# google/lasr

Hardware: AMD Instinct MI355X
Metric: rasterizer fwd+bwd frames/sec at 256x256, 2.3k faces (higher is better)
Workload: dtype f32

## Files before the change

### lasr_amd/csrc/sr_backward.h

```cpp
#pragma once
#include "sr_common.h"

namespace lasr {

constexpr bool BWD_FM = true;
constexpr int QCAP = 128;
constexpr int BWD_THREADS = 64;

template <bool LASR_FAST, int NCH, bool WIDE = false>
__global__ __launch_bounds__(BWD_THREADS)
__attribute__((amdgpu_waves_per_eu(LASR_FAST && NCH == 3 && !WIDE ? 6 : 1, LASR_FAST && NCH == 3 && !WIDE ? 7 : 8)))
void sr_backward_kernel(RasterArgs A, const float* __restrict__ colors,
                                                          const float* __restrict__ aggrs,
                                                          const float* __restrict__ gcolors,
                                                          float* __restrict__ gfaces, float* __restrict__ gtex)
{
    __shared__ unsigned int s_ring[BWD_THREADS / 64][QCAP];
    __shared__ __attribute__((aligned(16))) float s_rec[BWD_THREADS / 64][REC + (LASR_FAST ? BX : 0)];
    constexpr bool FM = BWD_FM;
    const Modes m = LASR_FAST ? Modes{2, 1, 2, 1, 1} : A.m;
    if (A.near_far_dev) { A.near = A.near_far_dev[0]; A.far = A.near_far_dev[1]; }
    const int lane = threadIdx.x & 63;
    unsigned int* ring = s_ring[threadIdx.x >> 6];
    int blk;
    {
        const int total = gridDim.x, per = total >> 3;
        blk = (total & 7) == 0 ? (blockIdx.x & 7) * per + (per - 1 - (blockIdx.x >> 3)) : total - 1 - blockIdx.x;
    }
    const int ext_src = LASR_FAST ? (int)k_bwd_ext_tbl[lane] : 0;
    const int gw = __builtin_amdgcn_readfirstlane((int)((blk * blockDim.x + threadIdx.x) >> 6));
    if (gw >= A.N * A.F) return;
    const int bn = face_div(gw, A.fdiv_m, A.fdiv_s), fn = gw - bn * A.F;
    const int IS = A.IS, P = IS * IS;
    const cptr_t rec = as_const(A.recs + (size_t)gw * REC);
    const cptr_t tex = as_const(A.textures + (size_t)gw * A.T * NCH);
    const int flags = __float_as_int(rec[R_FLAGS]);
    typedef const float __attribute__((address_space(3)))* lptr_t;
    if (LASR_FAST && (flags & 16)) {
        float* dst = s_rec[threadIdx.x >> 6];
        if (lane < REC) dst[lane] = A.recs[(size_t)gw * REC + lane];
        dst[REC + lane] = bwd_ext_word_tbl(A.recs + (size_t)gw * REC, flags, lane, ext_src);
        __builtin_amdgcn_wave_barrier();
    }
    const lptr_t lrec = (lptr_t)s_rec[threadIdx.x >> 6];

    const unsigned rlo = (unsigned)__float_as_int(rec[R_BB + 0]), rext = (unsigned)__float_as_int(rec[R_BB + 1]);
    const int x0 = (int)(rlo & 0xffff), r0 = (int)(rlo >> 16);
    const int bw = (int)(rext & 0xffff) + 1, bh = (int)(rext >> 16) + 1;
    const bool empty = rlo == 0xffffffffu;
    const int npx = empty ? 0 : bw * bh;

    float gv[9] = {0, 0, 0, 0, 0, 0, 0, 0, 0};
    constexpr int NGT = 3 * NCH < 18 ? 18 : 3 * NCH;
    constexpr int THIRD = NCH == 9 ? 18 : 0;
    float gt[NGT];
#pragma unroll
    for (int k = 0; k < NGT; k++) gt[k] = 0.f;
    const bool front = (flags & 8) != 0;
    const bool vertex_tex = (m.tex == 1);
    const int lim = (A.N * A.F - gw) * A.T;
    const bool use_far = (m.dist == 2) && (flags & 16);
    const float inv_is = A.inv_is;
    const bool pow2 = (IS & (IS - 1)) == 0;
    const float cx_a = A.cx_a, cx_b = A.cx_b, cy_b = A.cy_b;
    auto centre_x = [&](int xi) { return pow2 ? __builtin_fmaf((float)xi, cx_a, cx_b) : pix_center_p2(xi, IS, inv_is, pow2); };
    auto centre_y = [&](int row) { return pow2 ? __builtin_fmaf((float)row, -cx_a, cy_b) : pix_center_p2(IS - 1 - row, IS, inv_is, pow2); };
    float ld[9];
    const float far_t = A.far_t;
    if (use_far) {
#pragma unroll
        for (int k = 0; k < 3; k++) {
            const float h = __builtin_amdgcn_sqrtf(rec[R_HK2 + k]);
            ld[3 * k] = rec[R_INV + 3 * k] * h; ld[3 * k + 1] = rec[R_INV + 3 * k + 1] * h; ld[3 * k + 2] = rec[R_INV + 3 * k + 2] * h;
        }
    }
    const float tie_scale = rec[R_TIE];
    bool depth_safe = false;
    if (flags & 16) {
        const float z0 = rec[R_FACE + 2], z1 = rec[R_FACE + 5], z2 = rec[R_FACE + 8];
        const float zlo = fminf(fminf(z0, z1), z2), zhi = fmaxf(fmaxf(z0, z1), z2);
        depth_safe = zlo > 0.f && zlo * (1.f - 1e-4f) > A.near && zhi * (1.f + 1e-4f) < A.far;
    }
    constexpr int GC = 0, CO = 1, AG = 2;
    const unsigned P4 = (unsigned)P * 4u;

    int r = 0, c = 0;
    const int walk = __float_as_int(rec[15]);
    const int dr = empty ? 0 : walk >> 17, dc = empty ? 0 : 64 - dr * bw;
    if (!empty) { r = (lane * (walk & 0x1ffff)) >> 16; c = lane - r * bw; }

    int head = 0, tail = 0, base = 0;
    gplane_t pb[3];
    if (!WIDE) {
        pb[GC] = plane_base(gcolors, (size_t)bn * (NCH + 1), P);
        pb[CO] = plane_base(colors, (size_t)bn * (NCH + 1), P);
        pb[AG] = plane_base(aggrs, (size_t)bn * 2, P);
    }
    auto ld_plane = [&](const float* tensor, int which, int nplanes, int plane, int pn_, unsigned off_) -> float {
#if defined(LASR_BWD_ABL) && LASR_BWD_ABL == 3
        return 0.25f + 1e-3f * (float)(pn_ & 255) + 0.01f * (float)plane;
#endif
        if (WIDE) return tensor[((size_t)bn * nplanes + plane) * P + pn_];
        return ld_plane_at(pb[which], off_ + (unsigned)plane * P4);
    };
    while (true) {
        if (base < npx) {
            const int xi = x0 + c, row = r0 + r;
            const bool in_range = base + lane < npx;
            c += dc; r += dr;
            if (c >= bw) { c -= bw; r += 1; }
            base += 64;
            bool keep = in_range;
            if (use_far) {
                const float xp = __builtin_fmaf((float)xi, cx_a, cx_b), yp = __builtin_fmaf((float)row, -cx_a, cy_b);
                const float d0 = __builtin_fmaf(ld[0], xp, __builtin_fmaf(ld[1], yp, ld[2]));
                const float d1 = __builtin_fmaf(ld[3], xp, __builtin_fmaf(ld[4], yp, ld[5]));
                const float d2 = __builtin_fmaf(ld[6], xp, __builtin_fmaf(ld[7], yp, ld[8]));
                keep = in_range && !(fminf(fminf(d0, d1), d2) < far_t);
            }
            const unsigned long long mask = wave_mask(keep);
            if (keep) ring[(tail + bits_below_lane(mask)) & (QCAP - 1)] = (unsigned)xi | ((unsigned)row << 16);
            tail += __popcll(mask);
        }
        const int avail = tail - head;
        if (!(avail >= 64 || (base >= npx && avail > 0))) {
            if (base >= npx) break;
            continue;
        }
        __builtin_amdgcn_wave_barrier();
        const bool active = lane < avail;
        const unsigned int packed = ring[(head + lane) & (QCAP - 1)];
        head += min(avail, 64);
#if defined(LASR_BWD_ABL) && LASR_BWD_ABL == 1
        gv[0] += (float)packed;
        continue;
#endif
        if (!active) continue;
        const int xi = packed & 0xffff, row = packed >> 16;
        const int pn = row * IS + xi;
        unsigned po = (unsigned)pn << 2;
        const float xp = centre_x(xi), yp = centre_y(row);

        float w0, w1, w2;
        Frag fr;
        if (LASR_FAST && (flags & 16)) {
            if (!fragment_one_ext(lrec, lrec + REC, flags, A.thr, A.sigma, xp, yp, w0, w1, w2, fr, tie_scale)) continue;
        } else
        if (!fragment<FM, cptr_t, LASR_FAST>(rec, m.dist, A.thr, A.sigma, xp, yp, w0, w1, w2, fr)) continue;
        const float D = fr.D;
#if defined(LASR_BWD_ABL) && LASR_BWD_ABL == 2
        gv[0] += D + fr.dx + fr.dy + fr.t0 + fr.t1 + fr.t2 + fr.sign;
        continue;
#endif

        float Ca = ld_plane(gcolors, GC, NCH + 1, NCH, pn, po);
        if (m.alpha == 1) Ca = div_<FM>(Ca, (float)A.F);
        else if (m.alpha == 2) {
            const float a_out = ld_plane(colors, CO, NCH + 1, NCH, pn, po);
            Ca *= div_<FM>(1 - a_out, fmaxf(1 - D, 1e-6f));
        }
        float C = Ca;

        const float u0 = w0, u1 = w1, u2 = w2;
        if (vertex_tex) clip_normalise<FM, LASR_FAST>(w0, w1, w2); else clip_normalise<false>(w0, w1, w2);
        const float iz0r = rec[R_IZ + 0], iz1r = rec[R_IZ + 1], iz2r = rec[R_IZ + 2];
        const float q0 = w0 * iz0r, q1 = w1 * iz1r, q2 = w2 * iz2r;
        const float zp = LASR_FAST ? __builtin_amdgcn_rcpf(q0 + q1 + q2) : depth_at<FM>(rec, w0, w1, w2);
        if (!depth_safe) {
            float zc = zp;
            const float tol = 1e-4f * fabsf(zp);
            if (fabsf(zp - A.near) <= tol || fabsf(zp - A.far) <= tol) zc = depth_forward_exact(rec, xp, yp);
            if (zc < A.near || zc > A.far) continue;
        }

        float gz0 = 0, gz1 = 0, gz2 = 0;
        auto reenter = [&]() { if (!WIDE) asm volatile("" : "+v"(po)); };
        if (m.rgb == 0) {
            reenter();
            if ((float)fn == ld_plane(aggrs, AG, 2, 1, pn, po)) {
                reenter();
                float g[NCH];
#pragma unroll
                for (int k = 0; k < NCH; k++) g[k] = ld_plane(gcolors, GC, NCH + 1, k, pn, po);
                if (vertex_tex) {
#pragma unroll
                    for (int k = 0; k < NCH; k++) {
                        gt[k] += w0 * g[k]; gt[NCH + k] += w1 * g[k]; gt[2 * NCH + k] += w2 * g[k];
                    }
                } else {
                    const int j = surface_texel(w0, w1, A.res);
                    if (j >= 0 && j < A.T) {
                        float* gtp = gtex + (size_t)gw * A.T * 3 + 3 * j;
                        atomicAdd(gtp + 0, g[0]); atomicAdd(gtp + 1, g[1]); atomicAdd(gtp + 2, g[2]);
                    }
                }
            }
        } else if (front || m.double_side) {
            reenter();
            const float ssum = ld_plane(aggrs, AG, 2, 0, pn, po);
            const float smax = ld_plane(aggrs, AG, 2, 1, pn, po);
            const float zn = div_<FM>(A.far - zp, A.far - A.near);
            const float sm = div_<FM>(D * exp_<FM>(div_<FM>(zn - smax, A.gamma)), ssum);
            float g[NCH];
#pragma unroll
            for (int k = 0; k < NCH; k++) g[k] = ld_plane(gcolors, GC, NCH + 1, k, pn, po);
            if (vertex_tex) {
#pragma unroll
                for (int k = 0; k < NCH; k++) {
                    gt[k] += sm * (w0 * g[k]); gt[NCH + k] += sm * (w1 * g[k]); gt[2 * NCH + k] += sm * (w2 * g[k]);
                }
            } else {
                const int j = surface_texel(w0, w1, A.res);
                if (j >= 0 && j < A.T) {
                    float* gtp = gtex + (size_t)gw * A.T * 3 + 3 * j;
                    atomicAdd(gtp + 0, sm * g[0]); atomicAdd(gtp + 1, sm * g[1]); atomicAdd(gtp + 2, sm * g[2]);
                }
            }
            float Crgb = 0.f;
#pragma unroll
            for (int k = 0; k < NCH; k++)
                Crgb += g[k] * (sample_colour(tex, w0, w1, w2, A.res, k, m.tex, lim, NCH) - ld_plane(colors, CO, NCH + 1, k, pn, po));
            Crgb *= sm;
            C += div_<FM>(Crgb, D);
            const float Cz = div_<FM>(div_<FM>(Crgb, A.gamma), A.near - A.far) * zp * zp;
            if (LASR_FAST) {
                gz0 = Cz * q0 * iz0r; gz1 = Cz * q1 * iz1r; gz2 = Cz * q2 * iz2r;
            } else {
                const float iz0 = __builtin_amdgcn_rcpf(rec[R_FACE + 2]), iz1 = __builtin_amdgcn_rcpf(rec[R_FACE + 5]), iz2 = __builtin_amdgcn_rcpf(rec[R_FACE + 8]);
                gz0 = Cz * w0 * iz0 * iz0;
                gz1 = Cz * w1 * iz1 * iz1;
                gz2 = Cz * w2 * iz2 * iz2;
            }
        }

        C *= div_<FM>(D * (1 - D), A.sigma);
        float gx0 = 0, gy0 = 0, gx1 = 0, gy1 = 0, gx2 = 0, gy2 = 0;
        if (m.dist == 1) {
            const float t0 = fr.t0, t1 = fr.t1, t2 = fr.t2;
            const int p = t0 > t1 ? (t1 > t2 ? 2 : 1) : (t0 > t2 ? 2 : 0);
            const float ipx = rec[R_INV + 3 * p + 0], ipy = rec[R_INV + 3 * p + 1];
            const float dis = fr.dis;
            const float sc = 2.f * sqrtf(fabsf(dis));
            float gxy[3][2];
#pragma unroll
            for (int l = 0; l < 2; l++) {
                const float ipl = l == 0 ? ipx : ipy;
#pragma unroll
                for (int k = 0; k < 3; k++) {
                    float acc = 0.f;
                    acc += -ipl * rec[R_INV + 3 * k + 0] * xp;
                    acc += -ipl * rec[R_INV + 3 * k + 1] * yp;
                    acc += -ipl * rec[R_INV + 3 * k + 2] * 1.f;
                    gxy[k][l] = acc * C * sc;
                }
            }
            gx0 = gxy[0][0]; gy0 = gxy[0][1]; gx1 = gxy[1][0]; gy1 = gxy[1][1]; gx2 = gxy[2][0]; gy2 = gxy[2][1];
        } else if (m.dist == 2) {
            const float k2 = 2 * fr.sign * C;
            gx0 = k2 * (fr.t0 + u0) * fr.dx; gy0 = k2 * (fr.t0 + u0) * fr.dy;
            gx1 = k2 * (fr.t1 + u1) * fr.dx; gy1 = k2 * (fr.t1 + u1) * fr.dy;
            gx2 = k2 * (fr.t2 + u2) * fr.dx; gy2 = k2 * (fr.t2 + u2) * fr.dy;
        }
        gv[0] += gx0; gv[1] += gy0; gv[2] += gz0;
        gv[3] += gx1; gv[4] += gy1; gv[5] += gz1;
        gv[6] += gx2; gv[7] += gy2; gv[8] += gz2;
    }

    float v18[18], red[5];
    const int lane_row = lane >> 4;
    const int sub = lane_row == 0 ? 0 : lane_row == 1 ? 2 : lane_row == 2 ? 1 : 3;
    float* gf = gfaces + (size_t)gw * 9;
    float* gtp = gtex + (size_t)gw * 3 * NCH;
#pragma unroll
    for (int pass = 0; pass < (NCH > 3 ? 2 : 1); pass++) {
#pragma unroll
        for (int k = 0; k < 9; k++) {
            v18[k] = pass == 0 ? gv[k] : (vertex_tex ? gt[9 + k] : 0.f);
            v18[9 + k] = pass == 0 ? (vertex_tex ? gt[k] : 0.f) : (NCH == 9 && vertex_tex ? gt[THIRD + k] : 0.f);
        }
        wave_reduce18(v18, red);
        if ((lane & 15) == 15) {
#pragma unroll
            for (int i = 0; i < 5; i++) {
                if (i == 4 && (lane_row & 1)) continue;
                const int comp = i == 4 ? 16 + (lane_row >> 1) : 4 * i + sub;
                const bool ow = A.overwrite_grads && vertex_tex;
                if (pass == 0) {
                    if (comp < 9) gf[comp] = ow ? red[i] : gf[comp] + red[i];
                    else if (vertex_tex) gtp[comp - 9] = ow ? red[i] : gtp[comp - 9] + red[i];
                } else if ((comp < 9 || NCH == 9) && vertex_tex) gtp[9 + comp] = ow ? red[i] : gtp[9 + comp] + red[i];
            }
        }
    }
}

}
```

### lasr_amd/csrc/sr_device.h

```cpp
#pragma once
#include <hip/hip_runtime.h>

namespace lasr {

constexpr int REC = 48;

constexpr int R_BB = 0, R_FLAGS = 2, R_INV = 3, R_HK2 = 12, R_FACE = 16, R_DEN = 25, R_IDEN = 28, R_TIE = 31, R_E = 32, R_IZ = 41;

typedef const float __attribute__((address_space(4)))* cptr_t;
__device__ __forceinline__ cptr_t as_const(const float* p) { return (cptr_t)(unsigned long long)p; }

typedef const char __attribute__((address_space(1)))* gplane_t;
__device__ __forceinline__ gplane_t plane_base(const float* tensor, size_t plane, int P)
{
    unsigned long long u = (unsigned long long)(tensor + plane * (size_t)P);
    asm volatile("" : "+s"(u));
    return (gplane_t)u;
}
__device__ __forceinline__ float ld_plane_at(gplane_t base, unsigned byte_offset)
{
    return *(const float __attribute__((address_space(1)))*)(base + byte_offset);
}

struct Modes {
    int dist, rgb, alpha, tex, double_side;
};

__device__ __forceinline__ float pix_center(int i, int is)
{
    return (float)(2 * i + 1 - is) / (float)is;
}

__device__ __forceinline__ bool recip_safe(float b)
{
    const float m = fabsf(b);
    return m > 1e-18f && m < 1e18f;
}
__device__ __forceinline__ float div_by_recip(float a, float b, float y)
{
    float q = a * y;
    float e = __builtin_fmaf(-b, q, a);
    q = __builtin_fmaf(e, y, q);
    e = __builtin_fmaf(-b, q, a);
    return __builtin_fmaf(e, y, q);
}

__device__ __forceinline__ float recip_noscale(float x)
{
    float y = __builtin_amdgcn_rcpf(x);
    y = __builtin_fmaf(__builtin_fmaf(-x, y, 1.f), y, y);
    float q = y;
    q = __builtin_fmaf(__builtin_fmaf(-x, q, 1.f), y, q);
    return __builtin_fmaf(__builtin_fmaf(-x, q, 1.f), y, q);
}
__device__ __forceinline__ double recip64_noscale(double x)
{
    double y = __builtin_amdgcn_rcp(x);
    y = __builtin_fma(__builtin_fma(-x, y, 1.), y, y);
    y = __builtin_fma(__builtin_fma(-x, y, 1.), y, y);
    const double q = y;
    return __builtin_fma(__builtin_fma(-x, q, 1.), y, q);
}

__device__ __forceinline__ float max_finite(float a, float b)
{
    float r;
    asm("v_max_f32 %0, %1, %2" : "=v"(r) : "v"(a), "v"(b));
    return r;
}

typedef unsigned short u16x2_t __attribute__((ext_vector_type(2)));
__device__ __forceinline__ bool rect_has(int lo, int ext, int pxy)
{
    const u16x2_t d = __builtin_bit_cast(u16x2_t, pxy) - __builtin_bit_cast(u16x2_t, lo);
    const u16x2_t m = __builtin_elementwise_min(d, __builtin_bit_cast(u16x2_t, ext));
    return __builtin_bit_cast(int, m) == __builtin_bit_cast(int, d);
}

__device__ __forceinline__ int first_pixel_ge(float lo, int IS)
{
    if (lo != lo) return 0;
    const float e = ceilf((lo * (float)IS + (float)IS - 1.f) * 0.5f);
    int i = e < 0.f ? 0 : (e > (float)IS ? IS : (int)e);
    for (int k = 0; k < 4 && i > 0 && pix_center(i - 1, IS) >= lo; k++) i--;
    for (int k = 0; k < 4 && i < IS && pix_center(i, IS) < lo; k++) i++;
    return i;
}
__device__ __forceinline__ int last_pixel_le(float hi, int IS)
{
    if (hi != hi) return IS - 1;
    const float e = floorf((hi * (float)IS + (float)IS - 1.f) * 0.5f);
    int i = e < -1.f ? -1 : (e > (float)(IS - 1) ? IS - 1 : (int)e);
    for (int k = 0; k < 4 && i < IS - 1 && pix_center(i + 1, IS) <= hi; k++) i++;
    for (int k = 0; k < 4 && i >= 0 && pix_center(i, IS) > hi; k++) i--;
    return i;
}

__device__ __forceinline__ float pix_center_p2(int i, int is, float inv_is, bool pow2)
{
    return pow2 ? (float)(2 * i + 1 - is) * inv_is : pix_center(i, is);
}

__host__ __device__ __forceinline__ float near_tie_scale(float h2a, float h2b, float h2c);

__device__ __forceinline__ void build_record(const float* __restrict__ f, float* __restrict__ rec,
                                             short4* __restrict__ rect, float margin, int IS,
                                             float* __restrict__ info27)
{
    const float x0 = f[0], y0 = f[1], x1 = f[3], y1 = f[4], x2 = f[6], y2 = f[7];
    float adj[9];
    adj[0] = y1 - y2; adj[1] = x2 - x1; adj[2] = x1 * y2 - x2 * y1;
    adj[3] = y2 - y0; adj[4] = x0 - x2; adj[5] = x2 * y0 - x0 * y2;
    adj[6] = y0 - y1; adj[7] = x1 - x0; adj[8] = x0 * y1 - x1 * y0;
    float det = x2 * (y0 - y1) + x0 * (y1 - y2) + x1 * (y2 - y0);
    if (det > 0) { double d = (double)det; det = (float)(d > 1e-10 ? d : 1e-10); }
    else         { double d = (double)det; det = (float)(d < -1e-10 ? d : -1e-10); }
    float inv[9], sym[9];
#pragma unroll
    for (int k = 0; k < 9; k++) inv[k] = adj[k] / det;
#pragma unroll
    for (int j = 0; j < 3; j++)
#pragma unroll
        for (int k = 0; k < 3; k++) sym[3 * j + k] = f[3 * j] * f[3 * k] + f[3 * j + 1] * f[3 * k + 1] + 1;
    int flags = 0;
    {
        const float px[3] = {x0, x1, x2}, py[3] = {y0, y1, y2};
#pragma unroll
        for (int k = 0; k < 3; k++) {
            const int b = (k + 1) % 3, c = (k + 2) % 3;
            const bool obt = (px[b] - px[k]) * (px[c] - px[k]) + (py[b] - py[k]) * (py[c] - py[k]) < 0;
            if (obt && (flags & 7) == 0) flags |= 1 << k;
        }
    }
    if ((y2 - y0) * (x1 - x0) < (y1 - y0) * (x2 - x0)) flags |= 8;
#pragma unroll
    for (int k = 0; k < 9; k++) rec[R_FACE + k] = f[k];
#pragma unroll
    for (int k = 0; k < 9; k++) rec[R_INV + k] = inv[k];
#pragma unroll
    for (int k = 0; k < 3; k++) {
        const int b = (k + 1) % 3;
        float e[3];
#pragma unroll
        for (int j = 0; j < 3; j++) { e[j] = sym[3 * k + j] - sym[3 * b + j]; rec[R_E + 3 * k + j] = e[j]; }
        rec[R_DEN + k] = e[k] - e[b];
    }
    {
        const float det0 = x2 * (y0 - y1) + x0 * (y1 - y2) + x1 * (y2 - y0);
        const float px[3] = {x0, x1, x2}, py[3] = {y0, y1, y2};
        bool ok = true;
#pragma unroll
        for (int k = 0; k < 3; k++) {
            const int b = (k + 1) % 3, c = (k + 2) % 3;
            const float ex = px[c] - px[b], ey = py[c] - py[b];
            const float l2 = ex * ex + ey * ey;
            const float h2 = l2 > 0.f ? det0 * det0 / l2 : 0.f;
            rec[R_HK2 + k] = h2;
            ok = ok && (h2 > 1e-4f) && (h2 < 1e4f) && (l2 < 16.f);
        }
        if (ok) flags |= 16;
    }
    rec[R_FLAGS] = __int_as_float(flags);
    const float xmax = fmaxf(fmaxf(x0, x1), x2) + margin, xmin = fminf(fminf(x0, x1), x2) - margin;
    const float ymax = fmaxf(fmaxf(y0, y1), y2) + margin, ymin = fminf(fminf(y0, y1), y2) - margin;
    int px0 = first_pixel_ge(xmin, IS), px1 = last_pixel_le(xmax, IS);
    const int yi0 = first_pixel_ge(ymin, IS), yi1 = last_pixel_le(ymax, IS);
    int r0 = IS - 1 - yi1, r1 = IS - 1 - yi0;
    if (px0 > px1 || r0 > r1) { px0 = 32767; px1 = -1; r0 = 32767; r1 = -1; }
    *rect = make_short4((short)px0, (short)px1, (short)r0, (short)r1);
    if (px0 > px1) { rec[R_BB + 0] = __int_as_float(-1); rec[R_BB + 1] = __int_as_float(0); }
    else {
        rec[R_BB + 0] = __int_as_float((px0 & 0xffff) | (r0 << 16));
        rec[R_BB + 1] = __int_as_float(((px1 - px0) & 0xffff) | ((r1 - r0) << 16));
    }
    {
        bool ok = true;
#pragma unroll
        for (int k = 0; k < 3; k++) {
            const float d = rec[R_DEN + k], z = f[3 * k + 2];
            rec[R_IDEN + k] = 1.f / d;
            rec[R_IZ + k] = 1.f / z;
            ok = ok && recip_safe(d) && z >= 1e-6f && z <= 1e6f;
        }
#pragma unroll
        for (int k = 0; k < 9; k++) ok = ok && fabsf(inv[k]) < 1e30f;
        if (ok) rec[R_FLAGS] = __int_as_float(__float_as_int(rec[R_FLAGS]) | 32);
        {
            const int bw = px0 > px1 ? 1 : px1 - px0 + 1;
            const int mdiv = bw < 64 ? 65536 / bw + 1 : 0, dr = 64 / bw;
            rec[15] = __int_as_float(mdiv | (dr << 17));
        }
        rec[R_TIE] = (__float_as_int(rec[R_FLAGS]) & 16) ? near_tie_scale(rec[R_HK2], rec[R_HK2 + 1], rec[R_HK2 + 2]) : 0.f;
#pragma unroll
        for (int k = 44; k < REC; k++) rec[k] = 0.f;
    }
    if (info27) {
#pragma unroll
        for (int k = 0; k < 9; k++) { info27[k] = inv[k]; info27[9 + k] = sym[k]; }
        info27[18] = (flags & 1) ? 1.f : 0.f; info27[19] = (flags & 2) ? 1.f : 0.f; info27[20] = (flags & 4) ? 1.f : 0.f;
#pragma unroll
        for (int k = 21; k < 27; k++) info27[k] = 0.f;
    }
}

__device__ __forceinline__ bool inside_closed(float w0, float w1, float w2)
{
    return w0 <= 1 && w0 >= 0 && w1 <= 1 && w1 >= 0 && w2 <= 1 && w2 >= 0;
}

__device__ __forceinline__ void div3_shared(float& a0, float& a1, float& a2, float b)
{
    float y = __builtin_amdgcn_rcpf(b);
    y = __builtin_fmaf(__builtin_fmaf(-b, y, 1.f), y, y);
#define LASR_QUOT(a)                                                     \
    {                                                                    \
        float q = a * y;                                                 \
        q = __builtin_fmaf(__builtin_fmaf(-b, q, a), y, q);              \
        a = __builtin_fmaf(__builtin_fmaf(-b, q, a), y, q);              \
    }
    LASR_QUOT(a0) LASR_QUOT(a1) LASR_QUOT(a2)
#undef LASR_QUOT
}

template <bool FM = false, bool TAME = false>
__device__ __forceinline__ void clip_normalise(float& w0, float& w1, float& w2)
{
    if (TAME) {
        w0 = __builtin_amdgcn_fmed3f(w0, 0.f, 1.f);
        w1 = __builtin_amdgcn_fmed3f(w1, 0.f, 1.f);
        w2 = __builtin_amdgcn_fmed3f(w2, 0.f, 1.f);
    } else {
        w0 = fmaxf(fminf(w0, 1.f), 0.f);
        w1 = fmaxf(fminf(w1, 1.f), 0.f);
        w2 = fmaxf(fminf(w2, 1.f), 0.f);
    }
    const float s = fmaxf(w0 + w1 + w2, 1e-5f);
    if (FM) { const float r = __builtin_amdgcn_rcpf(s); w0 *= r; w1 *= r; w2 *= r; }
    else div3_shared(w0, w1, w2, s);
}

template <bool FM> __device__ __forceinline__ float div_(float a, float b)
{
    return FM ? a * __builtin_amdgcn_rcpf(b) : a / b;
}
__device__ __forceinline__ float exp_1ulp(float x)
{
    const float L2E_HI = 1.44269502162933349609375f, L2E_LO = 1.925963033500011e-8f;
    const float n = rintf(x * L2E_HI);
    const float f = __builtin_fmaf(x, L2E_LO, __builtin_fmaf(x, L2E_HI, -n));
    return ldexpf(__builtin_amdgcn_exp2f(f), (int)n);
}
template <bool FM> __device__ __forceinline__ float exp_(float x) { return FM ? __expf(x) : exp_1ulp(x); }
template <bool FM, bool NOSCALE = false> __device__ __forceinline__ float sigmoid_neg_(float neg_arg)
{
    if (FM) return __builtin_amdgcn_rcpf(1.f + __expf(neg_arg));
    if (NOSCALE) return (float)recip64_noscale(1. + (double)exp_1ulp(neg_arg));
    return (float)(1. / (1. + (double)exp_1ulp(neg_arg)));
}

template <int K, bool CLAMP, bool FM = false, bool MK = false, typename RP = cptr_t, bool IDEN = false>
__device__ __forceinline__ void edge_project(RP rec, float w0, float w1, float w2,
                                             float& u0, float& u1, float& u2)
{
#pragma clang fp contract(off)
    constexpr int B = (K + 1) % 3;
    const float e0 = rec[R_E + 3 * K + 0], e1 = rec[R_E + 3 * K + 1], e2 = rec[R_E + 3 * K + 2];
    const float eb = rec[R_E + 3 * K + B];
    const float num = w0 * e0 + w1 * e1 + w2 * e2 - eb;
    float ta = MK ? div_by_recip(num, rec[R_DEN + K], rec[R_IDEN + K])
                  : (FM && IDEN) ? num * rec[R_IDEN + K] : div_<FM>(num, rec[R_DEN + K]);
    float tb = 1 - ta;
    float tc = 0;
    if (CLAMP) {
        ta = fminf(fmaxf(ta, 0.f), 1.f);
        tb = fminf(fmaxf(tb, 0.f), 1.f);
    }
    float t[3];
    t[K] = ta; t[B] = tb; t[(K + 2) % 3] = tc;
    u0 = t[0] - w0; u1 = t[1] - w1; u2 = t[2] - w2;
}

struct Frag {
    float D;
    float sign, dx, dy;
    float t0, t1, t2;
    float dis;
    float narg;
};

template <bool FM = false, bool MK = false, typename RP = cptr_t, bool FWD = false, bool TAME = false, bool IDEN = false>
__device__ __forceinline__ bool euclid(RP rec, float xp, float yp,
                                       float w0, float w1, float w2, Frag& fr, float thr = 0.f)
{
#pragma clang fp contract(off)
    const float x0 = rec[R_FACE + 0], y0 = rec[R_FACE + 1], x1 = rec[R_FACE + 3], y1 = rec[R_FACE + 4], x2 = rec[R_FACE + 6], y2 = rec[R_FACE + 7];
    const bool inside = TAME ? (bool)((int)(fminf(fminf(w0, w1), w2) > 0) & (int)(fmaxf(fmaxf(w0, w1), w2) < 1))
                             : (w0 > 0 && w1 > 0 && w2 > 0 && w0 < 1 && w1 < 1 && w2 < 1);
    if (inside) {
        float best = 100000000.f, bx = 0, by = 0, b0 = 0, b1 = 0, b2 = 0;
        float u0, u1, u2;
#define LASR_TRY_EDGE(K)                                                          \
        edge_project<K, false, FM, MK, RP, IDEN>(rec, w0, w1, w2, u0, u1, u2);            \
        {                                                                         \
            const float px = u0 * x0 + u1 * x1 + u2 * x2;                         \
            const float py = u0 * y0 + u1 * y1 + u2 * y2;                         \
            const float d2 = px * px + py * py;                                   \
            if (d2 < best) { best = d2; bx = px; by = py; b0 = u0; b1 = u1; b2 = u2; } \
        }
        LASR_TRY_EDGE(0) LASR_TRY_EDGE(1) LASR_TRY_EDGE(2)
#undef LASR_TRY_EDGE
        if (FWD) { fr.narg = (-bx) * bx - by * by; return true; }
        fr.dx = bx; fr.dy = by; fr.t0 = b0; fr.t1 = b1; fr.t2 = b2; fr.sign = 1.f;
    } else {
        const int flags = __float_as_int(rec[R_FLAGS]);
        float u0, u1, u2;
        const bool n0 = w0 <= 0, n1 = w1 <= 0, n2 = w2 <= 0;
        bool o0 = false, o1 = false, o2 = false;
        if (flags & 7) {
            if (flags & 1) o0 = (xp - x0) * (x2 - x0) + (yp - y0) * (y2 - y0) > 0;
            if (flags & 2) o1 = (xp - x1) * (x0 - x1) + (yp - y1) * (y0 - y1) > 0;
            if (flags & 4) o2 = (xp - x2) * (x1 - x2) + (yp - y2) * (y1 - y2) > 0;
        }
        const bool c12 = n1 & n2, c20 = n2 & n0 & !n1, c01 = n0 & n1 & !n2;
        const bool e1 = (c20 & !o1) | (c01 & o2) | (n0 & !n1 & !n2);
        const bool e2 = (c01 & !o2) | (c12 & o0) | (n1 & !n0 & !n2);
        const bool e0 = !(e1 | e2);
        if (e0) edge_project<0, true, FM, MK, RP, IDEN>(rec, w0, w1, w2, u0, u1, u2);
        if (e1) edge_project<1, true, FM, MK, RP, IDEN>(rec, w0, w1, w2, u0, u1, u2);
        if (e2) edge_project<2, true, FM, MK, RP, IDEN>(rec, w0, w1, w2, u0, u1, u2);
        fr.dx = u0 * x0 + u1 * x1 + u2 * x2;
        fr.dy = u0 * y0 + u1 * y1 + u2 * y2;
        if (FWD) { fr.narg = fr.dx * fr.dx + fr.dy * fr.dy; return !(fr.narg >= thr); }
        fr.t0 = u0; fr.t1 = u1; fr.t2 = u2; fr.sign = -1.f;
    }
    return true;
}

__host__ __device__ constexpr unsigned edge_table(int obtuse_bits)
{
    unsigned t = 0;
    for (int over = 0; over < 2; over++)
        for (int idx = 0; idx < 8; idx++) {
            const bool n0 = idx & 1, n1 = idx & 2, n2 = idx & 4;
            const bool o0 = over && (obtuse_bits & 1), o1 = over && (obtuse_bits & 2), o2 = over && (obtuse_bits & 4);
            const bool c12 = n1 && n2, c20 = n2 && n0 && !n1, c01 = n0 && n1 && !n2;
            const bool e1 = (c20 && !o1) || (c01 && o2) || (n0 && !n1 && !n2);
            const bool e2 = (c01 && !o2) || (c12 && o0) || (n1 && !n0 && !n2);
            t |= (unsigned)((e1 ? 1 : 0) + (e2 ? 2 : 0)) << (2 * idx + 16 * over);
        }
    return t;
}

__host__ __device__ constexpr bool edge_table_matches()
{
    for (int v = 0; v < 4; v++) {
        const int ob = v == 0 ? 0 : 1 << (v - 1);
        const unsigned tbl = edge_table(ob);
        for (int over = 0; over < 2; over++)
            for (int idx = 0; idx < 8; idx++) {
                const int k = (int)((tbl >> (2 * idx + 16 * over)) & 3u);
                const bool n0 = idx & 1, n1 = idx & 2, n2 = idx & 4;
                const bool o0 = over && (ob & 1), o1 = over && (ob & 2), o2 = over && (ob & 4);
                const bool c12 = n1 & n2, c20 = n2 & n0 & !n1, c01 = n0 & n1 & !n2;
                const bool e1 = (c20 & !o1) | (c01 & o2) | (n0 & !n1 & !n2);
                const bool e2 = (c01 & !o2) | (c12 & o0) | (n1 & !n0 & !n2);
                const bool e0 = !(e1 | e2);
                if ((int)e0 + (int)e1 + (int)e2 != 1) return false;
                if (k != (e1 ? 1 : e2 ? 2 : 0)) return false;
                int a = -1;
                if (n1 && n2) { a = 0; if (o0) a = 2; }
                else if (n2 && n0) { a = 1; if (o1) a = 0; }
                else if (n0 && n1) { a = 2; if (o2) a = 1; }
                else if (n0) a = 1;
                else if (n1) a = 2;
                else if (n2) a = 0;
                if (a < 0) a = 0;
                if (k != a) return false;
                if (idx == 0 && k != 0) return false;
            }
    }
    return true;
}
static_assert(edge_table_matches(), "edge_table disagrees with euclid<>'s edge choice");

constexpr float NEAR_TIE = 0.985f;
constexpr float NEAR_TIE_ABS = 2.4e-6f;
__host__ __device__ __forceinline__ float near_tie_scale(float h2a, float h2b, float h2c)
{
    return 4.f * NEAR_TIE_ABS * NEAR_TIE_ABS / fminf(fminf(h2a, h2b), h2c);
}
__device__ __forceinline__ bool near_tie(float qlo, float qmid, float scale)
{
    const float gap = qmid - qlo;
    return (bool)((int)!(qlo < NEAR_TIE * qmid) | (int)!(gap * gap > scale * qmid));
}

constexpr int BX = 64, BX_STRIDE = 16, BX_OBT = 12;
typedef float f4_t __attribute__((ext_vector_type(4)));
typedef const float __attribute__((address_space(3)))* lds_cptr_t;
typedef const f4_t __attribute__((address_space(3)))* lds_c4ptr_t;
constexpr int BXT_ONE = 0x40, BXT_ZERO = 0x80, BXT_C = 0x100, BXT_O = 0x200;
static __constant__ constexpr unsigned short k_bwd_ext_tbl[BX] = {
    0x020, 0x021, 0x022, 0x021, 0x01c, 0x05c, 0x09c, 0x09c, 0x09c, 0x05c, 0x09c, 0x01c, 0x100, 0x101, 0x200, 0x201,
    0x023, 0x024, 0x025, 0x025, 0x01d, 0x09d, 0x05d, 0x09d, 0x09d, 0x09d, 0x05d, 0x01d, 0x01d, 0x01d, 0x01d, 0x01d,
    0x026, 0x027, 0x028, 0x026, 0x01e, 0x09e, 0x09e, 0x05e, 0x05e, 0x09e, 0x09e, 0x01e, 0x01e, 0x01e, 0x01e, 0x01e,
    0x029, 0x02a, 0x02b, 0x02d, 0x01f, 0x09f, 0x09f, 0x09f, 0x09f, 0x09f, 0x09f, 0x01f, 0x01f, 0x01f, 0x01f, 0x01f
};
__host__ __device__ constexpr int bwd_ext_formula(int L, int c)
{
    const int k = L >> 4, i = L & 15, o = c == 0 ? 2 : c - 1, kb = k == 2 ? 0 : k + 1;
    const bool obt = L >= BX_OBT && L < BX_OBT + 4;
    int ia = i < 3 ? R_E + 3 * k + i : i == 3 ? (k == 2 ? R_E + 6 : R_E + 4 * k + 1) : R_IDEN + k;
    ia = obt ? R_FACE + 3 * ((L & 2) ? o : c) + (L & 1) : ia;
    const int cst = (i >= 5 && i < 8) ? (i - 5 == k ? 1 : 0) : (i >= 8 && i < 11) ? (i - 8 == kb ? 1 : 0) : -1;
    return ia | ((obt && (L & 2)) ? 0x100 : 0) | ((cst + 1) << 9);
}
__host__ __device__ constexpr int bwd_ext_decode(int t, int c)
{
    const int o = c == 0 ? 2 : c - 1;
    const int ia = (t & 63) + ((t & BXT_O) ? R_FACE + 3 * o : (t & BXT_C) ? R_FACE + 3 * c : 0);
    const int cst = (t & BXT_ONE) ? 1 : (t & BXT_ZERO) ? 0 : -1;
    return ia | ((t & BXT_O) ? 0x100 : 0) | ((cst + 1) << 9);
}
__host__ __device__ constexpr bool bwd_ext_tbl_matches()
{
    for (int c = 0; c < 3; c++)
        for (int L = 0; L < BX; L++) {
            const int a = bwd_ext_formula(L, c), b = bwd_ext_decode(k_bwd_ext_tbl[L], c);
            if ((a >> 9) != (b >> 9) || ((a >> 9) == 0 && a != b)) return false;
        }
    return true;
}
static_assert(bwd_ext_tbl_matches(), "k_bwd_ext_tbl disagrees with the extension's layout (bwd_ext_formula)");
__device__ __forceinline__ float bwd_ext_word_tbl(const float* __restrict__ f, int flags, int L, int t)
{
    const int c = (flags & 1) ? 0 : (flags & 2) ? 1 : 2, o = c == 0 ? 2 : c - 1;
    const int cb = R_FACE + 3 * c, ob = R_FACE + 3 * o;
    const int ia = (t & 63) + ((t & BXT_O) ? ob : (t & BXT_C) ? cb : 0);
    const float a = f[ia], b = f[cb + (L & 1)];
    float v = (t & BXT_O) ? a - b : a;
    v = (t & BXT_ONE) ? 1.f : v;
    return (t & BXT_ZERO) ? 0.f : v;
}
__host__ __device__ constexpr unsigned edge_table_of_flags(int flags)
{
    return (flags & 1) ? edge_table(1) : (flags & 2) ? edge_table(2) : (flags & 4) ? edge_table(4) : edge_table(0);
}
__device__ __forceinline__ void euclid_one_ext(lds_cptr_t rec, lds_cptr_t ext, int flags, float xp, float yp, float w0, float w1, float w2,
                                               Frag& fr, float tie_scale)
{
#pragma clang fp contract(off)
    const float x0 = rec[R_FACE + 0], y0 = rec[R_FACE + 1], x1 = rec[R_FACE + 3], y1 = rec[R_FACE + 4], x2 = rec[R_FACE + 6], y2 = rec[R_FACE + 7];
    const bool inside = (bool)((int)(fminf(fminf(w0, w1), w2) > 0) & (int)(fmaxf(fmaxf(w0, w1), w2) < 1));
    const float q0 = w2 * w2 * rec[R_HK2 + 2], q1 = w0 * w0 * rec[R_HK2 + 0], q2 = w1 * w1 * rec[R_HK2 + 1];
    const float qlo = fminf(fminf(q0, q1), q2), qmid = __builtin_amdgcn_fmed3f(q0, q1, q2);
    const bool tie = (bool)((int)inside & (int)near_tie(qlo, qmid, tie_scale));
    float u0, u1, u2;
    if (tie) {
        float best = 100000000.f, bx = 0, by = 0, b0 = 0, b1 = 0, b2 = 0;
#define LASR_TRY_EDGE(K)                                                          \
        edge_project<K, false, true, false, lds_cptr_t, true>(rec, w0, w1, w2, u0, u1, u2);   \
        {                                                                         \
            const float px = u0 * x0 + u1 * x1 + u2 * x2;                         \
            const float py = u0 * y0 + u1 * y1 + u2 * y2;                         \
            const float d2 = px * px + py * py;                                   \
            if (d2 < best) { best = d2; bx = px; by = py; b0 = u0; b1 = u1; b2 = u2; } \
        }
        LASR_TRY_EDGE(0) LASR_TRY_EDGE(1) LASR_TRY_EDGE(2)
#undef LASR_TRY_EDGE
        fr.dx = bx; fr.dy = by; u0 = b0; u1 = b1; u2 = b2;
    } else {
        const bool i1 = (bool)((int)inside & (int)(q1 == qlo)), i2 = (bool)((int)inside & (int)(q2 == qlo));
        bool over = false;
        if (flags & 7) {
            const f4_t ob = *(lds_c4ptr_t)(ext + BX_OBT);
            over = (xp - ob.x) * ob.z + (yp - ob.y) * ob.w > 0;
        }
        const int sh = (w0 <= 0 ? 2 : 0) | (w1 <= 0 ? 4 : 0) | (w2 <= 0 ? 8 : 0) | (over ? 16 : 0);
        const int k = (int)__builtin_amdgcn_ubfe(edge_table_of_flags(flags), (unsigned)sh, 2u) | (i1 ? 1 : 0) | (i2 ? 2 : 0);
        const lds_cptr_t E = ext + BX_STRIDE * k;
        const f4_t ea = *(lds_c4ptr_t)E;
        const float num = w0 * ea.x + w1 * ea.y + w2 * ea.z - ea.w;
        float ta = num * E[4];
        float tb = 1 - ta;
        ta = fminf(fmaxf(ta, 0.f), 1.f);
        tb = fminf(fmaxf(tb, 0.f), 1.f);
        const f4_t fa = *(lds_c4ptr_t)(E + 4), fb = *(lds_c4ptr_t)(E + 8);
        const float t0 = __builtin_fmaf(tb, fb.x, ta * fa.y), t1 = __builtin_fmaf(tb, fb.y, ta * fa.z), t2 = __builtin_fmaf(tb, fb.z, ta * fa.w);
        u0 = t0 - w0; u1 = t1 - w1; u2 = t2 - w2;
        fr.dx = u0 * x0 + u1 * x1 + u2 * x2;
        fr.dy = u0 * y0 + u1 * y1 + u2 * y2;
    }
    fr.t0 = u0; fr.t1 = u1; fr.t2 = u2; fr.sign = inside ? 1.f : -1.f;
}

template <typename RP>
__device__ __forceinline__ void barycentric(RP rec, float xp, float yp, float& w0, float& w1, float& w2)
{
#pragma clang fp contract(off)
    w0 = rec[R_INV + 0] * xp + rec[R_INV + 1] * yp + rec[R_INV + 2];
    w1 = rec[R_INV + 3] * xp + rec[R_INV + 4] * yp + rec[R_INV + 5];
    w2 = rec[R_INV + 6] * xp + rec[R_INV + 7] * yp + rec[R_INV + 8];
}

template <bool FM = false, bool MK = false, typename RP = cptr_t, bool BT = false>
__device__ __forceinline__ bool fragment_w(RP rec, int dist, float thr, float sigma,
                                           float xp, float yp, float w0, float w1, float w2, Frag& fr,
                                           float inv_sigma = 0.f);

template <bool FM = false, typename RP = cptr_t, bool BT = false>
__device__ __forceinline__ bool fragment(RP rec, int dist, float thr, float sigma,
                                         float xp, float yp, float& w0, float& w1, float& w2, Frag& fr)
{
    barycentric(rec, xp, yp, w0, w1, w2);
    return fragment_w<FM, false, RP, BT>(rec, dist, thr, sigma, xp, yp, w0, w1, w2, fr);
}

template <bool FM, bool MK, typename RP, bool BT>
__device__ __forceinline__ bool fragment_w(RP rec, int dist, float thr, float sigma,
                                           float xp, float yp, float w0, float w1, float w2, Frag& fr, float inv_sigma)
{
#pragma clang fp contract(off)
    if (dist == 0) {
        if (!inside_closed(w0, w1, w2)) return false;
        fr.D = 1.f;
    } else if (dist == 1) {
        float d = w0 > w1 ? (w1 > w2 ? w2 : w1) : (w0 > w2 ? w2 : w0);
        d = d > 0 ? d * d : -(d * d);
        fr.dis = d; fr.t0 = w0; fr.t1 = w1; fr.t2 = w2;
        if (-d >= thr) return false;
        fr.D = sigmoid_neg_<FM>(MK ? div_by_recip(-d, sigma, inv_sigma) : div_<FM>(-d, sigma));
    } else if (!FM && MK) {
        if (!euclid<FM, MK, RP, true, true>(rec, xp, yp, w0, w1, w2, fr, thr)) return false;
        fr.D = sigmoid_neg_<FM, true>(div_by_recip(fr.narg, sigma, inv_sigma));
    } else {
        euclid<FM, MK, RP, false, (!FM && MK) || BT, BT>(rec, xp, yp, w0, w1, w2, fr);
        fr.dis = fr.dx * fr.dx + fr.dy * fr.dy;
        if (fr.sign < 0 && fr.dis >= thr) return false;
        fr.D = sigmoid_neg_<FM, (!FM && MK)>(MK ? div_by_recip(-fr.sign * fr.dis, sigma, inv_sigma) : div_<FM>(-fr.sign * fr.dis, sigma));
    }
    return true;
}

__device__ __forceinline__ bool fragment_one_ext(lds_cptr_t rec, lds_cptr_t ext, int flags, float thr, float sigma, float xp, float yp,
                                                 float& w0, float& w1, float& w2, Frag& fr, float tie_scale)
{
#pragma clang fp contract(off)
    barycentric(rec, xp, yp, w0, w1, w2);
    euclid_one_ext(rec, ext, flags, xp, yp, w0, w1, w2, fr, tie_scale);
    fr.dis = fr.dx * fr.dx + fr.dy * fr.dy;
    if (fr.sign < 0 && fr.dis >= thr) return false;
    fr.D = sigmoid_neg_<true>(div_<true>(-fr.sign * fr.dis, sigma));
    return true;
}

template <bool FM = false, bool MK = false, typename RP = cptr_t>
__device__ __forceinline__ float depth_at(RP rec, float c0, float c1, float c2)
{
    if (MK) {
        const float s = div_by_recip(c0, rec[R_FACE + 2], rec[R_IZ + 0]) + div_by_recip(c1, rec[R_FACE + 5], rec[R_IZ + 1]) +
                        div_by_recip(c2, rec[R_FACE + 8], rec[R_IZ + 2]);
        return recip_noscale(s);
    }
    return div_<FM>(1.f, div_<FM>(c0, rec[R_FACE + 2]) + div_<FM>(c1, rec[R_FACE + 5]) + div_<FM>(c2, rec[R_FACE + 8]));
}

template <typename RP>
__device__ __forceinline__ float depth_forward_exact(RP rec, float xp, float yp)
{
#pragma clang fp contract(off)
    float w0 = rec[R_INV + 0] * xp + rec[R_INV + 1] * yp + rec[R_INV + 2];
    float w1 = rec[R_INV + 3] * xp + rec[R_INV + 4] * yp + rec[R_INV + 5];
    float w2 = rec[R_INV + 6] * xp + rec[R_INV + 7] * yp + rec[R_INV + 8];
    w0 = fmaxf(fminf(w0, 1.f), 0.f);
    w1 = fmaxf(fminf(w1, 1.f), 0.f);
    w2 = fmaxf(fminf(w2, 1.f), 0.f);
    const float s = fmaxf(w0 + w1 + w2, 1e-5f);
    w0 = w0 / s; w1 = w1 / s; w2 = w2 / s;
    return 1.f / (w0 / rec[R_FACE + 2] + w1 / rec[R_FACE + 5] + w2 / rec[R_FACE + 8]);
}

__device__ __forceinline__ int surface_texel(float c0, float c1, int res)
{
    const int ix = (int)(c0 * res), iy = (int)(c1 * res);
    if ((c0 + c1) * res - ix - iy <= 1) return iy * res + ix;
    return (res - 1 - iy) * res + (res - 1 - ix);
}

template <typename TP>
__device__ __forceinline__ float sample_colour(TP tex, float c0, float c1, float c2,
                                               int res, int ch, int tex_type, int lim, int nch = 3)
{
    if (tex_type == 0) {
        const int j = max(min(surface_texel(c0, c1, res), lim - 1), 0);
        return tex[j * 3 + ch];
    }
    return c0 * tex[ch] + c1 * tex[nch + ch] + c2 * tex[2 * nch + ch];
}

__device__ __forceinline__ unsigned long long wave_mask(bool c) { return __builtin_amdgcn_ballot_w64(c); }
__device__ __forceinline__ int bits_below_lane(unsigned long long m)
{
    return (int)__builtin_amdgcn_mbcnt_hi((unsigned)(m >> 32), __builtin_amdgcn_mbcnt_lo((unsigned)m, 0u));
}

__device__ __forceinline__ float wave_sum_to_lane63(float v)
{
#define LASR_DPP_ADD(ctrl, rmask, bmask)                                                              \
    v += __int_as_float(__builtin_amdgcn_update_dpp(0, __float_as_int(v), ctrl, rmask, bmask, false))
    LASR_DPP_ADD(0x111, 0xf, 0xf);
    LASR_DPP_ADD(0x112, 0xf, 0xf);
    LASR_DPP_ADD(0x114, 0xf, 0xe);
    LASR_DPP_ADD(0x118, 0xf, 0xc);
    LASR_DPP_ADD(0x142, 0xa, 0xf);
    LASR_DPP_ADD(0x143, 0xc, 0xf);
#undef LASR_DPP_ADD
    return v;
}

__device__ __forceinline__ float swap_add32(float a, float b)
{
    const auto r = __builtin_amdgcn_permlane32_swap(__float_as_uint(a), __float_as_uint(b), false, false);
    return __uint_as_float(r[0]) + __uint_as_float(r[1]);
}
__device__ __forceinline__ float swap_add16(float a, float b)
{
    const auto r = __builtin_amdgcn_permlane16_swap(__float_as_uint(a), __float_as_uint(b), false, false);
    return __uint_as_float(r[0]) + __uint_as_float(r[1]);
}
__device__ __forceinline__ float row_sum_to_lane15(float v)
{
#define LASR_DPP_ADD(ctrl, bmask) \
    v += __int_as_float(__builtin_amdgcn_update_dpp(0, __float_as_int(v), ctrl, 0xf, bmask, false))
    LASR_DPP_ADD(0x111, 0xf);
    LASR_DPP_ADD(0x112, 0xf);
    LASR_DPP_ADD(0x114, 0xe);
    LASR_DPP_ADD(0x118, 0xc);
#undef LASR_DPP_ADD
    return v;
}
__device__ __forceinline__ void wave_reduce18(const float (&v)[18], float (&out)[5])
{
    float s[9];
#pragma unroll
    for (int i = 0; i < 9; i++) s[i] = swap_add32(v[2 * i], v[2 * i + 1]);
#pragma unroll
    for (int i = 0; i < 4; i++) out[i] = row_sum_to_lane15(swap_add16(s[2 * i], s[2 * i + 1]));
    out[4] = row_sum_to_lane15(swap_add16(s[8], 0.f));
}

}
```

Measured before the change: 119,800.

## Precompute sqrt and packed depth range in face record; hoist backward constants

Per-face square roots of HK2 and a packed 16-bit depth-range test are moved into the face record during setup, so the backward kernel no longer computes them per wave. The per-pixel aggregation path replaces several divisions and exp with precomputed reciprocals and an exp2 scaled by log2(e), and folds the softmax weight into the gradient colours once. This cuts per-pixel ALU work in the hot backward loop, at the cost of slightly different rounding and a conservative truncated depth-range check.

```diff
diff --git a/lasr_amd/csrc/sr_backward.h b/lasr_amd/csrc/sr_backward.h
--- a/lasr_amd/csrc/sr_backward.h
+++ b/lasr_amd/csrc/sr_backward.h
@@ -70,17 +70,15 @@
     if (use_far) {
 #pragma unroll
         for (int k = 0; k < 3; k++) {
-            const float h = __builtin_amdgcn_sqrtf(rec[R_HK2 + k]);
+            const float h = rec[R_HS + k];
             ld[3 * k] = rec[R_INV + 3 * k] * h; ld[3 * k + 1] = rec[R_INV + 3 * k + 1] * h; ld[3 * k + 2] = rec[R_INV + 3 * k + 2] * h;
         }
     }
+    const float inv_fmn = div_<FM>(1.f, A.far - A.near), inv_gamma = div_<FM>(1.f, A.gamma);
+    const float zn_a = -inv_fmn, zn_b = A.far * inv_fmn;
+    const float ex_k = inv_gamma * 1.44269504088896341f, cz_k = -(inv_gamma * inv_fmn);
     const float tie_scale = rec[R_TIE];
-    bool depth_safe = false;
-    if (flags & 16) {
-        const float z0 = rec[R_FACE + 2], z1 = rec[R_FACE + 5], z2 = rec[R_FACE + 8];
-        const float zlo = fminf(fminf(z0, z1), z2), zhi = fmaxf(fmaxf(z0, z1), z2);
-        depth_safe = zlo > 0.f && zlo * (1.f - 1e-4f) > A.near && zhi * (1.f + 1e-4f) < A.far;
-    }
+    const bool depth_safe = (flags & 16) && depth_range_inside(rec[R_ZR], A.near, A.far);
     constexpr int GC = 0, CO = 1, AG = 2;
     const unsigned P4 = (unsigned)P * 4u;
 
@@ -199,30 +197,29 @@
             reenter();
             const float ssum = ld_plane(aggrs, AG, 2, 0, pn, po);
             const float smax = ld_plane(aggrs, AG, 2, 1, pn, po);
-            const float zn = div_<FM>(A.far - zp, A.far - A.near);
-            const float sm = div_<FM>(D * exp_<FM>(div_<FM>(zn - smax, A.gamma)), ssum);
-            float g[NCH];
-#pragma unroll
-            for (int k = 0; k < NCH; k++) g[k] = ld_plane(gcolors, GC, NCH + 1, k, pn, po);
+            const float zn = zp * zn_a + zn_b;
+            const float sm = div_<FM>(D * __builtin_amdgcn_exp2f((zn - smax) * ex_k), ssum);
+            float sg[NCH];
+#pragma unroll
+            for (int k = 0; k < NCH; k++) sg[k] = sm * ld_plane(gcolors, GC, NCH + 1, k, pn, po);
             if (vertex_tex) {
 #pragma unroll
                 for (int k = 0; k < NCH; k++) {
-                    gt[k] += sm * (w0 * g[k]); gt[NCH + k] += sm * (w1 * g[k]); gt[2 * NCH + k] += sm * (w2 * g[k]);
+                    gt[k] += w0 * sg[k]; gt[NCH + k] += w1 * sg[k]; gt[2 * NCH + k] += w2 * sg[k];
                 }
             } else {
                 const int j = surface_texel(w0, w1, A.res);
                 if (j >= 0 && j < A.T) {
                     float* gtp = gtex + (size_t)gw * A.T * 3 + 3 * j;
-                    atomicAdd(gtp + 0, sm * g[0]); atomicAdd(gtp + 1, sm * g[1]); atomicAdd(gtp + 2, sm * g[2]);
+                    atomicAdd(gtp + 0, sg[0]); atomicAdd(gtp + 1, sg[1]); atomicAdd(gtp + 2, sg[2]);
                 }
             }
             float Crgb = 0.f;
 #pragma unroll
             for (int k = 0; k < NCH; k++)
-                Crgb += g[k] * (sample_colour(tex, w0, w1, w2, A.res, k, m.tex, lim, NCH) - ld_plane(colors, CO, NCH + 1, k, pn, po));
-            Crgb *= sm;
+                Crgb += sg[k] * (sample_colour(tex, w0, w1, w2, A.res, k, m.tex, lim, NCH) - ld_plane(colors, CO, NCH + 1, k, pn, po));
             C += div_<FM>(Crgb, D);
-            const float Cz = div_<FM>(div_<FM>(Crgb, A.gamma), A.near - A.far) * zp * zp;
+            const float Cz = (Crgb * cz_k) * (zp * zp);
             if (LASR_FAST) {
                 gz0 = Cz * q0 * iz0r; gz1 = Cz * q1 * iz1r; gz2 = Cz * q2 * iz2r;
             } else {
@@ -257,9 +254,10 @@
             gx0 = gxy[0][0]; gy0 = gxy[0][1]; gx1 = gxy[1][0]; gy1 = gxy[1][1]; gx2 = gxy[2][0]; gy2 = gxy[2][1];
         } else if (m.dist == 2) {
             const float k2 = 2 * fr.sign * C;
-            gx0 = k2 * (fr.t0 + u0) * fr.dx; gy0 = k2 * (fr.t0 + u0) * fr.dy;
-            gx1 = k2 * (fr.t1 + u1) * fr.dx; gy1 = k2 * (fr.t1 + u1) * fr.dy;
-            gx2 = k2 * (fr.t2 + u2) * fr.dx; gy2 = k2 * (fr.t2 + u2) * fr.dy;
+            const float kx = k2 * fr.dx, ky = k2 * fr.dy;
+            gx0 = (fr.t0 + u0) * kx; gy0 = (fr.t0 + u0) * ky;
+            gx1 = (fr.t1 + u1) * kx; gy1 = (fr.t1 + u1) * ky;
+            gx2 = (fr.t2 + u2) * kx; gy2 = (fr.t2 + u2) * ky;
         }
         gv[0] += gx0; gv[1] += gy0; gv[2] += gz0;
         gv[3] += gx1; gv[4] += gy1; gv[5] += gz1;
diff --git a/lasr_amd/csrc/sr_device.h b/lasr_amd/csrc/sr_device.h
--- a/lasr_amd/csrc/sr_device.h
+++ b/lasr_amd/csrc/sr_device.h
@@ -5,7 +5,7 @@
 
 constexpr int REC = 48;
 
-constexpr int R_BB = 0, R_FLAGS = 2, R_INV = 3, R_HK2 = 12, R_FACE = 16, R_DEN = 25, R_IDEN = 28, R_TIE = 31, R_E = 32, R_IZ = 41;
+constexpr int R_BB = 0, R_FLAGS = 2, R_INV = 3, R_HK2 = 12, R_FACE = 16, R_DEN = 25, R_IDEN = 28, R_TIE = 31, R_E = 32, R_IZ = 41, R_HS = 44, R_ZR = 47;
 
 typedef const float __attribute__((address_space(4)))* cptr_t;
 __device__ __forceinline__ cptr_t as_const(const float* p) { return (cptr_t)(unsigned long long)p; }
@@ -102,6 +102,20 @@
 }
 
 __host__ __device__ __forceinline__ float near_tie_scale(float h2a, float h2b, float h2c);
+
+__device__ __forceinline__ float pack_depth_range(float z0, float z1, float z2)
+{
+    const float zlo = fminf(fminf(z0, z1), z2), zhi = fmaxf(fmaxf(z0, z1), z2);
+    const float lo = zlo * (1.f - 1e-4f), hi = zhi * (1.f + 1e-4f);
+    const unsigned lo16 = zlo > 0.f ? (unsigned)__float_as_int(lo) >> 16 : 0xff80u;
+    const unsigned hi16 = hi > 0.f ? ((unsigned)__float_as_int(hi) + 0xffffu) >> 16 : 0x7f80u;
+    return __int_as_float((int)(lo16 | hi16 << 16));
+}
+__device__ __forceinline__ bool depth_range_inside(float zr, float near, float far)
+{
+    const unsigned u = (unsigned)__float_as_int(zr);
+    return __int_as_float((int)(u << 16)) > near && __int_as_float((int)(u & 0xffff0000u)) < far;
+}
 
 __device__ __forceinline__ void build_record(const float* __restrict__ f, float* __restrict__ rec,
                                              short4* __restrict__ rect, float margin, int IS,
@@ -191,8 +205,12 @@
             rec[15] = __int_as_float(mdiv | (dr << 17));
         }
         rec[R_TIE] = (__float_as_int(rec[R_FLAGS]) & 16) ? near_tie_scale(rec[R_HK2], rec[R_HK2 + 1], rec[R_HK2 + 2]) : 0.f;
-#pragma unroll
-        for (int k = 44; k < REC; k++) rec[k] = 0.f;
+        {
+            const bool well = (__float_as_int(rec[R_FLAGS]) & 16) != 0;
+#pragma unroll
+            for (int k = 0; k < 3; k++) rec[R_HS + k] = well ? __builtin_amdgcn_sqrtf(rec[R_HK2 + k]) : 0.f;
+            rec[R_ZR] = pack_depth_range(f[2], f[5], f[8]);
+        }
     }
     if (info27) {
 #pragma unroll
```

New measurement: 121,300 (median of 6 runs). 1.01x the previous value.
